# liuyuan-pal/NeRO

Measured on AMD Instinct MI355X. Metric: training rays/sec (Stage-I shape, 128 samples/ray), higher is better.
Workload: dtype f32 (dense layers: fp32 operands carried as exact / block-scaled 16-bit plane pairs or triples on the bf16/fp16 matrix pipe with fp32 accumulation, fp32-grade error; modes {'fwd': 'f16x3', 'tan': 'f16x3', 'bwd': 'f16x3', 'dw': 'f16x3'}); 1 GPU; GlossySynthetic 'bell' Stage-I shape, 4096 rays x (64+64+32) samples per GPU, training-schedule step 25000; rays_per_gpu=4096, parallelism=dp1, optimizer=adam(fused), streams=3, f16_paired_mask=3, fg_table=reference asset (tests/golden/fg_lut_ref.npz)

## Files before the change

### nero_amd/chain.py

```python
import ctypes as C
import os
import math

import torch

from . import _lib as L




_MODE_NAMES = {'f32': L.GEMM_F32, 'bf16x6': L.GEMM_BF16X6, 'f16x3': L.GEMM_F16X3}
_F16 = (L.GEMM_F16X3,)
_DEFAULT = {'fwd': 'f16x3', 'tan': 'f16x3', 'bwd': 'f16x3', 'dw': 'f16x3'}


def _resolve(mode, k):
    if mode not in _MODE_NAMES:
        raise ValueError(f"NERO_GEMM{'_' + k.upper()}: unknown arithmetic {mode!r} (one of {sorted(_MODE_NAMES)}; 'f16x3p' is not an arithmetic any more: "
                         "NERO_F16_PAIRED selects the workgroup organisation, DESIGN.md 9.3)")
    return _MODE_NAMES[mode]


GEMM_MODE = {k: _resolve(os.environ.get('NERO_GEMM_' + k.upper(), os.environ.get('NERO_GEMM', _DEFAULT[k])), k)
             for k in ('fwd', 'tan', 'bwd', 'dw')}
# ... 141 lines not shown
                e['hw'] = 4 * L.HID
                e['hb'] = 4
            sizes.append(e)
        return sizes

    def pack_floats(self):
        return sum(sum(e.values()) for e in self._sizes())

    def pack(self, buf=None, run=True):
        sizes = self._sizes()
        total = sum(sum(e.values()) for e in sizes)
        if buf is None:
            buf = torch.zeros(total, dtype=torch.float32, device=self.device)
        assert buf.numel() >= total
        off = 0
        packed = []
        jobs = []

        def job(kind, W, out, nrows, ld, col0, ncols, transpose, kpad, nt_count, scale=1.0):
            j = L.PackJob()
            j.W, j.out, j.kind, j.nrows, j.ld, j.col0, j.ncols = W.data_ptr(), out.data_ptr(), kind, nrows, ld, col0, ncols
            j.transpose, j.kpad, j.nt_count, j.scale = transpose, kpad, nt_count, scale
            jobs.append((j, W))

        for (d, h), e in zip(self.entries, sizes):
            p = {}
            for k, n in e.items():
                p[k] = buf[off:off + n] if n else None
                off += n
            if d is not None:
                W = d.W.detach()
                assert W.stride(1) == 1
                nt = _tiles(d.n_out)
                for key, c0, kc in (('fm', d.main_c0, d.k_main), ('fa', d.aux_c0, d.k_aux)):
                    if kc and key in p:
                        job(1, W, p[key], d.n_out, W.stride(0), c0, kc, 0, _r8(kc), nt, d.scale)
                for key, c0, kc in (('bm', d.main_c0, d.k_main), ('ba', d.aux_c0, d.k_aux)):
                    if kc and key in p:
                        job(1, W, p[key], d.n_out, W.stride(0), c0, kc, 1, _r8(d.n_out), _tiles(kc), d.scale)
                for key, c0, kc in (('sfm', d.main_c0, d.k_main), ('sfa', d.aux_c0, d.k_aux)):
                    if kc and key in p:
                        job(0, W, p[key], d.n_out, W.stride(0), c0, kc, 0, _r16(kc), nt, d.scale)
                for key, c0, kc in (('sbm', d.main_c0, d.k_main), ('sba', d.aux_c0, d.k_aux)):
                    if kc and key in p:
                        job(0, W, p[key], d.n_out, W.stride(0), c0, kc, 1, _r16(d.n_out), _tiles(kc), d.scale)
                for key, c0, kc in (('hfm', d.main_c0, d.k_main), ('hfa', d.aux_c0, d.k_aux)):
                    if kc and key in p:
                        job(3, W, p[key], d.n_out, W.stride(0), c0, kc, 0, _r16(kc), nt, d.scale)
                for key, c0, kc in (('hbm', d.main_c0, d.k_main), ('hba', d.aux_c0, d.k_aux)):
                    if kc and key in p:
                        job(3, W, p[key], d.n_out, W.stride(0), c0, kc, 1, _rev_k(d.n_out), _tiles(kc), d.scale)
                if d.b is not None:
                    b = d.b.detach()
                    job(2, b, p['bias'], 1, d.n_out, 0, d.n_out, 0, 32 * nt, 0)
            if h is not None:
                Wh = h.W.detach()
                assert Wh.stride(1) == 1
                job(2, Wh, p['hw'], h.n_head, Wh.stride(0), 0, h.k, 0, L.HID, 0)
                if h.b is not None:
                    job(2, h.b.detach(), p['hb'], 1, h.n_head, 0, h.n_head, 0, 4, 0)
            packed.append(p)
        self._packed, self._buf = packed, buf
        if not run:
            return jobs
        run_pack_jobs(jobs)
        return self

    def forward(self, init, aux, n_rows, save=True):
        assert self._packed is not None
        rp = row_pad(n_rows)
        ch = L.FwdChain()
        ch.init, ch.ld_init, ch.k_init = L.ptr(init), (init.stride(0) if init is not None else 0), self.k_init
        ch.aux, ch.ld_aux, ch.k_aux = L.ptr(aux), (aux.stride(0) if aux is not None else 0), self.k_aux
        ch.n_layers, ch.aux_wide = len(self.entries), int(self.aux_wide)
        split = GEMM_MODE['fwd'] != L.GEMM_F32
        fkeys = {L.GEMM_F32: ('fm', 'fa'), L.GEMM_BF16X6: ('sfm', 'sfa'), L.GEMM_F16X3: ('hfm', 'hfa')}[GEMM_MODE['fwd']]
        ch.gemm_mode = GEMM_MODE['fwd']
        ch.macs_per_row = float(sum(d.n_out * (d.k_main + d.k_aux) for d, _ in self.entries if d is not None))
        if init is not None:
            assert init.shape[0] >= rp and init.shape[1] >= self.k_init
        if aux is not None:
            assert aux.shape[0] >= rp and aux.shape[1] >= self.k_aux
        nd = len(self.dense_idx)
        last_dense = self.dense_idx[-1] if nd else -1
        saves, heads = [None] * len(self.entries), {}
        n_save = sum(1 for i in self.dense_idx if save or i == last_dense)
        sbuf = torch.empty((n_save, rp, L.HID), dtype=torch.float32, device=self.device)
        si = 0
        masks = [None] * len(self.entries)
        relu_idx = [i for i in self.dense_idx if save and self.entries[i][0].act == L.ACT_RELU] if GEMM_MODE['fwd'] in _F16 else []
        mbuf = torch.empty((len(relu_idx), rp, 8), dtype=torch.int32, device=self.device) if relu_idx else None
        for k, i in enumerate(relu_idx):
            masks[i] = mbuf[k]
        for i, ((d, h), p) in enumerate(zip(self.entries, self._packed)):
            fl = ch.layer[i]
            if h is not None:
                ho = torch.empty((rp, 4), dtype=torch.float32, device=self.device)
                heads[i] = ho
                fl.head_w, fl.head_b, fl.head_out = p['hw'].data_ptr(), p['hb'].data_ptr(), ho.data_ptr()
                fl.n_head, fl.head_k = h.n_head, (h.k + 3) // 4 * 4
            if d is not None:
                rk = _r16 if split else _r8
                fl.w_main = L.ptr(p.get(fkeys[0]))
                fl.w_aux = L.ptr(p.get(fkeys[1]))
                fl.bias = p['bias'].data_ptr()
                fl.k_main, fl.k_aux = (rk(d.k_main) if d.k_main else 0), (rk(d.k_aux) if d.k_aux else 0)
                fl.n_tiles, fl.act = _tiles(d.n_out), d.act
                if save or i == last_dense:
                    saves[i] = sbuf[si]
                    si += 1
                    fl.save = saves[i].data_ptr()
                if masks[i] is not None:
                    fl.relu_mask = masks[i].data_ptr()
        L.check(L.lib.nero_mlp_forward(C.byref(ch), n_rows, L.stream_ptr()))
        if MASK_CAPTURE is not None and relu_idx:
            MASK_CAPTURE.append({'k_init': self.k_init, 'k_aux': self.k_aux, 'aux_wide': bool(self.aux_wide), 'n_rows': n_rows,
                                 'n_out': [d.n_out if d is not None else 0 for d, _ in self.entries], 'masks': masks})
        return {'saves': saves, 'heads': heads, 'masks': masks, '_keep': (init, aux)}

    def backward(self, fwd, n_rows, dy=None, head_dys=None, need_dinit=False, need_daux=False, injs=None,
                 dinit_out=None, accumulate_dinit=False, skip_last_dense=False):
        head_dys = head_dys or {}
        injs = injs or {}
        rp = row_pad(n_rows)
        saves = fwd['saves']
        ch = L.BwdChain()
        ch.n_layers, ch.aux_wide = len(self.entries), 0
        split = GEMM_MODE['bwd'] != L.GEMM_F32
        bkeys = {L.GEMM_F32: ('bm', 'ba'), L.GEMM_BF16X6: ('sbm', 'sba'), L.GEMM_F16X3: ('hbm', 'hba')}[GEMM_MODE['bwd']]
        ch.gemm_mode = GEMM_MODE['bwd']
        rk = _r16 if split else _r8
        last = len(self.entries) - 1
        if dy is not None:
            ch.dy, ch.ld_dy = dy.data_ptr(), dy.stride(0)
            d_last = self.entries[last][0]
            ch.k_dy = _r8(d_last.n_out) if d_last is not None else L.HID
            assert dy.shape[1] >= ch.k_dy
        d_init = d_aux = None
        if need_dinit:
            d_init = dinit_out if dinit_out is not None else torch.empty((rp, self.k_init), dtype=torch.float32, device=self.device)
            ch.d_init, ch.ld_dinit, ch.accumulate_dinit = d_init.data_ptr(), d_init.stride(0), int(accumulate_dinit)
        if need_daux:
            d_aux = torch.zeros((rp, self.k_aux), dtype=torch.float32, device=self.device)
            ch.d_aux, ch.ld_daux = d_aux.data_ptr(), d_aux.stride(0)
        deltas = {}
        n_delta = len(self.dense_idx)
        dbuf = torch.empty((n_delta, rp, L.HID), dtype=torch.float32, device=self.device)
        prev_dense = {}
        pd = None
        for i, (d, h) in enumerate(self.entries):
            prev_dense[i] = pd
            if d is not None:
                pd = i
        for k, i in enumerate(self.dense_idx):
            deltas[i] = dbuf[k]
        for i, ((d, h), p) in enumerate(zip(self.entries, self._packed)):
            bl = ch.layer[i]
            j = prev_dense[i]
            if d is not None and not (skip_last_dense and i == last):
                bl.w_main_t = L.ptr(p.get(bkeys[0]))
                bl.w_aux_t = L.ptr(p.get(bkeys[1])) if need_daux else None
                bl.n_out = _rev_k(d.n_out) if GEMM_MODE['bwd'] in _F16 else rk(d.n_out)
                bl.k_main_tiles = _tiles(d.k_main) if d.k_main else 0
                bl.k_aux_tiles = _tiles(d.k_aux) if d.k_aux else 0
            else:
                bl.n_out = 0
                bl.k_main_tiles = _tiles(self.entries[j][0].n_out)
# ... 86 lines not shown
```

### nero_amd/csrc/chain_host.h

```cpp
#pragma once
#include <hip/hip_runtime_api.h>
#include <math.h>
#include <stdio.h>
#include <string.h>
#include <new>
#include <vector>
#include "../../include/nero_hip.h"

int nero_fail(int code, const char* msg);
int nero_check_launch(const char* what);
bool nero_prof_is_on();

namespace {

constexpr int MAXL = NERO_MAX_LAYERS;
inline int r8(int x) { return (x + 7) / 8 * 8; }
inline int r16(int x) { return (x + 15) / 16 * 16; }
inline int tiles(int x) { return (x + 31) / 32; }
inline int rpad(int n) { return NERO_ROW_PAD(n); }
inline int rev_k(int n_out) { return (n_out > 128 && n_out <= 256) ? 256 : r16(n_out); }
inline bool is_f16(int m) { return m == NERO_GEMM_F16X3; }

struct Arena {
    char* base = nullptr;
// ... 37 lines not shown
    float *bias = nullptr, *hfm = nullptr, *hfa = nullptr, *hbm = nullptr, *hba = nullptr, *hw = nullptr, *hb = nullptr;
};
struct Fwd {
    float* saves[MAXL]; uint32_t* masks[MAXL]; float* heads[MAXL];
    Fwd() { for (int i = 0; i < MAXL; ++i) { saves[i] = nullptr; masks[i] = nullptr; heads[i] = nullptr; } }
};
struct Bwd {
    const float* deltas[MAXL]; int ld_delta[MAXL];
    float* d_init = nullptr; int ld_dinit = 0; float* d_aux = nullptr; int ld_daux = 0;
    Bwd() { for (int i = 0; i < MAXL; ++i) { deltas[i] = nullptr; ld_delta[i] = NERO_HID; } }
};
struct Second { const float* D1 = nullptr; int ldd1 = 0; const float* B1m = nullptr; int ldb1m = 0; const float* B1a = nullptr; int ldb1a = 0; };

struct Modes { int fwd, tan, bwd, dw; };

struct Chain {
    std::vector<Entry> e;
    int k_init = 0, k_aux = 0, aux_wide = 0;
    int n() const { return (int)e.size(); }
    int last_dense() const { int l = -1; for (int i = 0; i < n(); ++i) if (e[i].d.has) l = i; return l; }

    size_t pack_floats() const {
        size_t t = 0;
        for (const Entry& x : e) {
            if (x.d.has) {
                const Dense& d = x.d;
                const int nt = tiles(d.n_out);
                t += 32 * nt;
                if (d.k_main) t += 64 + (size_t)(r16(d.k_main) / 16) * nt * 512 + 64 + (size_t)(rev_k(d.n_out) / 16) * tiles(d.k_main) * 512;
                if (d.k_aux) t += 64 + (size_t)(r16(d.k_aux) / 16) * nt * 512 + 64 + (size_t)(rev_k(d.n_out) / 16) * tiles(d.k_aux) * 512;
            }
            if (x.h.has) t += 4 * NERO_HID + 4;
        }
        return t;
    }
    void pack(float*& buf, std::vector<nero_pack_job>& jobs) {
        auto job = [&](int kind, const float* W, float* out, int nrows, int ld, int col0, int ncols, int transpose, int kpad, int nt_count, float scale) {
            nero_pack_job j;
            j.W = W; j.out = out; j.kind = kind; j.nrows = nrows; j.ld = ld; j.col0 = col0; j.ncols = ncols; j.transpose = transpose;
            j.kpad = kpad; j.nt_count = nt_count; j.scale = scale; j.pad_ = 0;
            jobs.push_back(j);
        };
        for (Entry& x : e) {
            if (x.d.has) {
                const Dense& d = x.d;
                const int nt = tiles(d.n_out);
                x.bias = buf; buf += 32 * nt;
                x.hfm = x.hfa = x.hbm = x.hba = nullptr;
                if (d.k_main) {
                    x.hfm = buf; buf += 64 + (size_t)(r16(d.k_main) / 16) * nt * 512;
                    x.hbm = buf; buf += 64 + (size_t)(rev_k(d.n_out) / 16) * tiles(d.k_main) * 512;
                    job(3, d.W, x.hfm, d.n_out, d.ldw, d.main_c0, d.k_main, 0, r16(d.k_main), nt, d.scale);
                    job(3, d.W, x.hbm, d.n_out, d.ldw, d.main_c0, d.k_main, 1, rev_k(d.n_out), tiles(d.k_main), d.scale);
                }
                if (d.k_aux) {
                    x.hfa = buf; buf += 64 + (size_t)(r16(d.k_aux) / 16) * nt * 512;
                    x.hba = buf; buf += 64 + (size_t)(rev_k(d.n_out) / 16) * tiles(d.k_aux) * 512;
                    job(3, d.W, x.hfa, d.n_out, d.ldw, d.aux_c0, d.k_aux, 0, r16(d.k_aux), nt, d.scale);
                    job(3, d.W, x.hba, d.n_out, d.ldw, d.aux_c0, d.k_aux, 1, rev_k(d.n_out), tiles(d.k_aux), d.scale);
                }
                if (d.b) job(2, d.b, x.bias, 1, d.n_out, 0, d.n_out, 0, 32 * nt, 0, 1.f);
            }
            if (x.h.has) {
                x.hw = buf; buf += 4 * NERO_HID;
                x.hb = buf; buf += 4;
                job(2, x.h.W, x.hw, x.h.n_head, x.h.ldw, 0, x.h.k, 0, NERO_HID, 0, 1.f);
                if (x.h.b) job(2, x.h.b, x.hb, 1, x.h.n_head, 0, x.h.n_head, 0, 4, 0, 1.f);
            }
        }
    }

    int forward(Arena& A, const Modes& M, const float* init, int ld_init, const float* aux, int ld_aux, int n_rows, bool save, Fwd& F,
                void* stream) const {
        const int rp = rpad(n_rows);
        nero_fwd_chain ch;
        memset(&ch, 0, sizeof(ch));
        ch.init = init; ch.ld_init = init ? ld_init : 0; ch.k_init = k_init;
        ch.aux = aux; ch.ld_aux = aux ? ld_aux : 0; ch.k_aux = k_aux;
        ch.n_layers = n(); ch.aux_wide = aux_wide;
        ch.gemm_mode = M.fwd;
        double macs = 0.0;
        for (const Entry& x : e) if (x.d.has) macs += (double)x.d.n_out * (x.d.k_main + x.d.k_aux);
        ch.macs_per_row = macs;
        const int ld = last_dense();
        for (int i = 0; i < n(); ++i) {
            const Entry& x = e[i];
            nero_fwd_layer& fl = ch.layer[i];
            if (x.h.has) {
                F.heads[i] = A.f32((size_t)rp * 4);
                fl.head_w = x.hw; fl.head_b = x.hb; fl.head_out = F.heads[i];
                fl.n_head = x.h.n_head; fl.head_k = (x.h.k + 3) / 4 * 4;
            }
            if (x.d.has) {
                const Dense& d = x.d;
                fl.w_main = x.hfm; fl.w_aux = x.hfa; fl.bias = x.bias;
                fl.k_main = d.k_main ? r16(d.k_main) : 0; fl.k_aux = d.k_aux ? r16(d.k_aux) : 0;
                fl.n_tiles = tiles(d.n_out); fl.act = d.act;
                if (save || i == ld) { F.saves[i] = A.f32((size_t)rp * NERO_HID); fl.save = F.saves[i]; }
                if (save && d.act == NERO_ACT_RELU) { F.masks[i] = reinterpret_cast<uint32_t*>(A.i32((size_t)rp * 8)); fl.relu_mask = F.masks[i]; }
            }
        }
        if (A.failed) return nero_fail(NERO_ERR_ARG, "nero_stage1: workspace too small");
        LAUNCH(nero_mlp_forward(&ch, n_rows, stream));
        return NERO_OK;
    }

    int backward(Arena& A, const Modes& M, const Fwd& F, int n_rows, const float* dy, int ld_dy, const float* const* head_dys ,
                 bool need_dinit, bool need_daux, const float* const* injs , float* dinit_out, int ld_dinit_out,
                 bool accumulate_dinit, bool skip_last_dense, Bwd& B, void* stream,
                 const float* const* inj_adots = nullptr ) const {
        const int rp = rpad(n_rows), last = n() - 1;
        nero_bwd_chain ch;
        memset(&ch, 0, sizeof(ch));
        ch.n_layers = n(); ch.aux_wide = 0; ch.gemm_mode = M.bwd;
        if (dy) {
            ch.dy = dy; ch.ld_dy = ld_dy;
            ch.k_dy = e[last].d.has ? r8(e[last].d.n_out) : NERO_HID;
        }
        if (need_dinit) {
            if (dinit_out) { B.d_init = dinit_out; B.ld_dinit = ld_dinit_out; }
            else { B.d_init = A.f32((size_t)rp * k_init); B.ld_dinit = k_init; }
            ch.d_init = B.d_init; ch.ld_dinit = B.ld_dinit; ch.accumulate_dinit = accumulate_dinit ? 1 : 0;
        }
        if (need_daux) {
            B.d_aux = A.f32((size_t)rp * k_aux); B.ld_daux = k_aux;
            if (!A.dry && !A.failed) (void)hipMemsetAsync(B.d_aux, 0, (size_t)rp * k_aux * 4, (hipStream_t)stream);
            ch.d_aux = B.d_aux; ch.ld_daux = k_aux;
        }
        int prev_dense[MAXL];
        int pd = -1;
        for (int i = 0; i < n(); ++i) { prev_dense[i] = pd; if (e[i].d.has) pd = i; }
        float* dw[MAXL];
        for (int i = 0; i < n(); ++i) {
            dw[i] = nullptr;
            if (e[i].d.has) { dw[i] = A.f32((size_t)rp * NERO_HID); B.deltas[i] = dw[i]; B.ld_delta[i] = NERO_HID; }
        }
        double macs = 0.0;
        for (int i = 0; i < n(); ++i) {
            const Entry& x = e[i];
            nero_bwd_layer& bl = ch.layer[i];
            const int j = prev_dense[i];
            if (x.d.has && !(skip_last_dense && i == last)) {
                const Dense& d = x.d;
                bl.w_main_t = x.hbm;
                bl.w_aux_t = need_daux ? x.hba : nullptr;
                bl.n_out = rev_k(d.n_out);
                bl.k_main_tiles = d.k_main ? tiles(d.k_main) : 0;
                bl.k_aux_tiles = d.k_aux ? tiles(d.k_aux) : 0;
                const bool first = j < 0;
                if (first && !need_dinit) macs += (need_daux && d.k_aux) ? (double)d.n_out * d.k_aux : 0.0;
                else macs += (double)d.n_out * (d.k_main + (need_daux ? d.k_aux : 0));
            } else {
                bl.n_out = 0;
                bl.k_main_tiles = j >= 0 ? tiles(e[j].d.n_out) : 0;
            }
            if (x.h.has && head_dys && head_dys[i]) { bl.head_w = x.hw; bl.head_dy = head_dys[i]; bl.n_head = x.h.n_head; }
            if (j >= 0) {
                bl.a_prev = F.saves[j];
                bl.act_prev = e[j].d.act;
                if (F.masks[j]) bl.mask_prev = F.masks[j];
                bl.delta_prev = dw[j];
                if (injs && injs[j]) { bl.inj = injs[j]; if (inj_adots && inj_adots[j]) bl.inj_adot = inj_adots[j]; }
            }
        }
        if (e[last].d.has && !skip_last_dense) { B.deltas[last] = dy; B.ld_delta[last] = ld_dy; }
        ch.macs_per_row = macs;
        if (A.failed) return nero_fail(NERO_ERR_ARG, "nero_stage1: workspace too small");
// ... 151 lines not shown
```

### nero_amd/csrc/mlp_f16_util.h

```cpp
#pragma once

#ifdef F16_PHASE_TIMING
__device__ unsigned long long g_phase[16];
#define PH_DECL long long ph_t = clock64(), ph_acc[8] = {0, 0, 0, 0, 0, 0, 0, 0}
#define PH(k) do { __builtin_amdgcn_sched_barrier(0); const long long t_ = clock64(); ph_acc[k] += t_ - ph_t; ph_t = t_; __builtin_amdgcn_sched_barrier(0); } while (0)
#define PH_PARAM , long long& ph_t, long long (&ph_acc)[8]
#define PH_ARG , ph_t, ph_acc
#define PH_END do { if (threadIdx.x == 0) for (int k_ = 0; k_ < 8; ++k_) atomicAdd(&g_phase[k_], (unsigned long long)ph_acc[k_]); } while (0)
#else
#define PH_PARAM
#define PH_ARG
#define PH_DECL
#define PH(k)
#define PH_END
#endif

typedef _Float16 f16x8 __attribute__((ext_vector_type(8)));
typedef _Float16 f16x2 __attribute__((ext_vector_type(2)));
typedef float f32x2 __attribute__((ext_vector_type(2)));
typedef float f32x16 __attribute__((ext_vector_type(16)));

constexpr float BETA = 100.0f;
constexpr int SA = 528;
constexpr int PLANE_A = 64 * SA;
// ... 303 lines not shown
                     "global_load_dwordx4 %2, %4, %6\n\tglobal_load_dwordx4 %3, %4, %6 offset:1024"
    if (ORDER_MEM) asm volatile(NERO_W2Q_ASM : "=&v"(o.ah), "=&v"(o.al), "=&v"(o.bh), "=&v"(o.bl) : "v"(voff), "s"(p0), "s"(p1) : "memory");
    else asm volatile(NERO_W2Q_ASM : "=&v"(o.ah), "=&v"(o.al), "=&v"(o.bh), "=&v"(o.bl) : "v"(voff), "s"(p0), "s"(p1));
#undef NERO_W2Q_ASM
}
static_assert(WQ_PLANE_BYTES == 1024, "offset:1024 in load_w2q");
template <int N> __device__ __forceinline__ void wait_vm() { asm volatile("s_waitcnt vmcnt(%0)" : : "n"(N)); }
__device__ __forceinline__ void landed_w2q(WQ2& w) {
    NERO_FENCE();
    asm volatile("" : "+v"(w.ah), "+v"(w.al), "+v"(w.bh), "+v"(w.bl));
}
__device__ __forceinline__ void ops_compute2q(f32x16 (&aH0)[2], f32x16 (&aH1)[2], const WQ2& w, const XF& x) {
    NERO_MFH(aH0[0], w.al, x.xh0); NERO_MFH(aH0[1], w.al, x.xh1);
    NERO_MFH(aH0[0], w.ah, x.xl0); NERO_MFH(aH0[1], w.ah, x.xl1);
    NERO_MFH(aH0[0], w.ah, x.xh0); NERO_MFH(aH0[1], w.ah, x.xh1);
    NERO_MFH(aH1[0], w.bl, x.xh0); NERO_MFH(aH1[1], w.bl, x.xh1);
    NERO_MFH(aH1[0], w.bh, x.xl0); NERO_MFH(aH1[1], w.bh, x.xl1);
    NERO_MFH(aH1[0], w.bh, x.xh0); NERO_MFH(aH1[1], w.bh, x.xh1);
}
__device__ __forceinline__ void prefill_w2q(WQ2& r0, WQ2& r1, unsigned voff, const char* s0, const char* s1) {
    load_w2q<0, true>(r0, voff, s0, s1);
    load_w2q<1, true>(r1, voff, s0, s1);
    NERO_FENCE();
}
constexpr int PRE_STORES = 2 * 2 * (32 / SCRP_ROWS) * (SCRP_ROWS / 8);
template <int N>
__device__ __forceinline__ void gemm_f16x3_dual_fixed(f32x16 (&aH0)[2], f32x16 (&aH1)[2], unsigned voff, const char* s0, const char* s1,
                                                      const char* xp, int half_bytes, int plane_bytes, WQ2& r0, WQ2& r1, bool stores_behind) {
    static_assert(N >= 3, "ring of three");
    WQ2 r2;
    XF x[2];
    load_x(x[0], xp, half_bytes, plane_bytes, 0);
    NERO_FENCE();
    static_for<0, N>([&](auto cc) {
        constexpr int c = cc.value;
        auto slot = [&](auto k) -> WQ2& { if constexpr (k.value % 3 == 0) return r0; else if constexpr (k.value % 3 == 1) return r1; else return r2; };
        if constexpr (c + 2 < N) load_w2q<c + 2, false>(slot(IC<c + 2>{}), voff, s0, s1);
        if constexpr (c + 1 < N) load_x(x[(c + 1) & 1], xp, half_bytes, plane_bytes, c + 1);
        NERO_FENCE();
        constexpr int later = 4 * ((c + 1 < N ? 1 : 0) + (c + 2 < N ? 1 : 0));
        if (c < 2 && stores_behind) wait_vm<later + PRE_STORES>();
        else wait_vm<later>();
        landed_w2q(slot(cc));
        ops_compute2q(aH0, aH1, slot(cc), x[c & 1]);
        NERO_FENCE();
    });
}

struct WQ1 { u32x4 h, l; };
template <int C> __device__ __forceinline__ void load_w1q(WQ1& o, unsigned voff, const char* s) {
    const char* p = s + C * WQ_STEP_BYTES;
    asm volatile("s_nop 4\n\tglobal_load_dwordx4 %0, %2, %3\n\tglobal_load_dwordx4 %1, %2, %3 offset:1024"
                 : "=&v"(o.h), "=&v"(o.l) : "v"(voff), "s"(p));
}
__device__ __forceinline__ void landed_w1q(WQ1& w) {
    NERO_FENCE();
    asm volatile("" : "+v"(w.h), "+v"(w.l));
}
template <int N>
__device__ __forceinline__ void gemm_f16x3_single_fixed(f32x16 (&aH)[2], unsigned voff, const char* s, const char* xp, int half_bytes,
                                                        int plane_bytes) {
    constexpr int WD = 3, WN = WD + 1;
    static_assert(N > WD, "ring of four");
    WQ1 w[WN];
    XF x[2];
    static_for<0, WD>([&](auto cc) { load_w1q<cc.value>(w[cc.value], voff, s); });
    load_x(x[0], xp, half_bytes, plane_bytes, 0);
    NERO_FENCE();
    static_for<0, N>([&](auto cc) {
        constexpr int c = cc.value;
        if constexpr (c + WD < N) load_w1q<c + WD>(w[(c + WD) % WN], voff, s);
        if constexpr (c + 1 < N) load_x(x[(c + 1) & 1], xp, half_bytes, plane_bytes, c + 1);
        NERO_FENCE();
        constexpr int later = 2 * ((c + 1 < N ? 1 : 0) + (c + 2 < N ? 1 : 0) + (c + 3 < N ? 1 : 0));
        wait_vm<later>();
        landed_w1q(w[c % WN]);
        NERO_MFH(aH[0], w[c % WN].l, x[c & 1].xh0); NERO_MFH(aH[1], w[c % WN].l, x[c & 1].xh1);
        NERO_MFH(aH[0], w[c % WN].h, x[c & 1].xl0); NERO_MFH(aH[1], w[c % WN].h, x[c & 1].xl1);
        NERO_MFH(aH[0], w[c % WN].h, x[c & 1].xh0); NERO_MFH(aH[1], w[c % WN].h, x[c & 1].xh1);
        NERO_FENCE();
    });
}

__device__ __forceinline__ void zero2(f32x16 (&acc)[2]) {
#pragma unroll
    for (int r = 0; r < 2; ++r)
#pragma unroll
        for (int v = 0; v < 16; ++v) acc[r][v] = 0.f;
}

template <int ACT>
__device__ __forceinline__ void fwd_values(const f32x16 (&aH)[2], const float4 (&bq)[4], const float (&U)[2], float4 (&val)[2][4],
                                           float (&m)[2]) {
#pragma unroll
    for (int r = 0; r < 2; ++r) {
        m[r] = 0.f;
#pragma unroll
        for (int g = 0; g < 4; ++g) {
            float4 v;
            v.x = act_fwd<ACT>(fmaf(aH[r][4 * g], U[r], bq[g].x));
            v.y = act_fwd<ACT>(fmaf(aH[r][4 * g + 1], U[r], bq[g].y));
            v.z = act_fwd<ACT>(fmaf(aH[r][4 * g + 2], U[r], bq[g].z));
            v.w = act_fwd<ACT>(fmaf(aH[r][4 * g + 3], U[r], bq[g].w));
            val[r][g] = v;
            m[r] = fmaxf(m[r], amax4(v));
        }
    }
}

__device__ __forceinline__ float max_xor32(float m) {
    const auto r = __builtin_amdgcn_permlane32_swap(__float_as_uint(m), __float_as_uint(m), false, false);
    return fmaxf(__uint_as_float(r[0]), __uint_as_float(r[1]));
}
__device__ __forceinline__ unsigned other_half(unsigned v, int h) {
    const auto r = __builtin_amdgcn_permlane32_swap(v, v, false, false);
    return h ? r[0] : r[1];
}
template <int CTRL> __device__ __forceinline__ float dpp_f32(float v) {
    return __uint_as_float(__builtin_amdgcn_update_dpp(0u, __float_as_uint(v), CTRL, 0xf, 0xf, true));
}
__device__ __forceinline__ float max_4lanes(float m) { m = fmaxf(m, dpp_f32<0xB1>(m)); return fmaxf(m, dpp_f32<0x4E>(m)); }
__device__ __forceinline__ float max_8lanes(float m) { m = max_4lanes(m); return fmaxf(m, dpp_f32<0x141>(m)); }
__device__ __forceinline__ float sum_8lanes(float s) { s += dpp_f32<0xB1>(s); s += dpp_f32<0x4E>(s); return s + dpp_f32<0x141>(s); }

__device__ __forceinline__ void publish_rowmax(float* rmax, float m0, float m1, int wave, int i, int h) {
    m0 = max_xor32(m0);
    m1 = max_xor32(m1);
    if (h == 0) { rmax[i * 8 + wave] = m0; rmax[(32 + i) * 8 + wave] = m1; }
}
__device__ __forceinline__ float row_max8(const float* rmax, int row) {
    const float4 a = *reinterpret_cast<const float4*>(rmax + row * 8);
    const float4 b = *reinterpret_cast<const float4*>(rmax + row * 8 + 4);
    return fmaxf(fmaxf(fmaxf(a.x, a.y), fmaxf(a.z, a.w)), fmaxf(fmaxf(b.x, b.y), fmaxf(b.z, b.w)));
}

template <int ACT, bool HEAD, bool PRE>
__device__ __forceinline__ void bwd_values(const float4 (&gq)[2][4], const float4 (&pa)[2][4], size_t goff, bool has_inj,
                                           const nero_bwd_layer& L, int row0, int i, int fbase, int n_rows, float4 (&val)[2][4],
                                           float (&m)[2], const float4 (&ijp)[2][4]) {
    const int nh = L.n_head;
    float4 gs[2][4];
#pragma unroll
    for (int r = 0; r < 2; ++r)
#pragma unroll
        for (int g = 0; g < 4; ++g) gs[r][g] = gq[r][g];
    if (HEAD) {
        float dj[2][4];
#pragma unroll
        for (int r = 0; r < 2; ++r) {
            const float4 dyh = *reinterpret_cast<const float4*>(L.head_dy + (size_t)(row0 + 32 * r + i) * 4);
            dj[r][0] = dyh.x; dj[r][1] = dyh.y; dj[r][2] = dyh.z; dj[r][3] = dyh.w;
        }
#pragma unroll
        for (int g = 0; g < 4; ++g) {
            float4 hw[4];
#pragma unroll
            for (int j = 0; j < 4; ++j) hw[j] = *reinterpret_cast<const float4*>(L.head_w + (j < nh ? j : 0) * NERO_HID + fbase + 8 * g);
#pragma unroll
            for (int r = 0; r < 2; ++r)
#pragma unroll
                for (int j = 0; j < 4; ++j)
                    if (j < nh) {
                        gs[r][g].x = fmaf(dj[r][j], hw[j].x, gs[r][g].x); gs[r][g].y = fmaf(dj[r][j], hw[j].y, gs[r][g].y);
                        gs[r][g].z = fmaf(dj[r][j], hw[j].z, gs[r][g].z); gs[r][g].w = fmaf(dj[r][j], hw[j].w, gs[r][g].w);
                    }
            __builtin_amdgcn_sched_barrier(0);
// ... 48 lines not shown
```

### nero_amd/csrc/mlp_f16x3.hip

```cpp
#include <hip/hip_runtime.h>
#include <stdint.h>
#include <stdlib.h>
#include "../../include/nero_hip.h"
#include "common.h"
#include "mlp_split.h"

namespace {

#include "mlp_f16_util.h"


__device__ __forceinline__ void acc_to_global(float* scr, const float4 (&q)[4], float* __restrict__ gblock, int lane) {
    const int i = lane & 31, h = lane >> 5;
#pragma unroll
    for (int g = 0; g < 4; ++g) *reinterpret_cast<float4*>(scr + i * SCR_LD + 8 * g + 4 * h) = q[g];
    __builtin_amdgcn_wave_barrier();
#pragma unroll
    for (int p = 0; p < 4; ++p)
        store_ws4(gblock + (size_t)(8 * p + (lane >> 3)) * NERO_HID + 4 * (lane & 7),
                  *reinterpret_cast<const float4*>(scr + (8 * p + (lane >> 3)) * SCR_LD + 4 * (lane & 7)));
    __builtin_amdgcn_wave_barrier();
}

template <int NV>
__device__ __forceinline__ void tile_request(float4 (&v)[NV], const float* __restrict__ src, int ld, int k, int row0, int n_rows, int tid) {
    const int r = tid >> 3, q = tid & 7;
    int gr = row0 + r;
    gr = gr < n_rows ? gr : n_rows - 1;
    const float* rowp = src + (size_t)gr * ld;
#pragma unroll
    for (int j = 0; j < NV; ++j) {
        const int c4 = 4 * (q + 8 * j);
        v[j] = make_float4(0.f, 0.f, 0.f, 0.f);
        if (c4 < k) v[j] = *reinterpret_cast<const float4*>(rowp + c4);
    }
}
template <int NV>
__device__ __forceinline__ void tile_commit(char* planes, int stride, int plane_bytes, float* rs, const float4 (&v)[NV], int k, int tid) {
    const int r = tid >> 3, q = tid & 7;
    const int k16 = (k + 15) & ~15, q4 = k16 >> 2;
    float m = 0.f;
#pragma unroll
    for (int j = 0; j < NV; ++j) m = fmaxf(m, fmaxf(fmaxf(fabsf(v[j].x), fabsf(v[j].y)), fmaxf(fabsf(v[j].z), fabsf(v[j].w))));
    m = max_8lanes(m);
    const int e = scale_exp(m);
    const float inv = pow2i(-e);
#pragma unroll
    for (int j = 0; j < NV; ++j) {
        const int c4 = 4 * (q + 8 * j);
        if (q + 8 * j < q4) {
            const float4 s = make_float4(v[j].x * inv, v[j].y * inv, v[j].z * inv, v[j].w * inv);
            store_planes4h(planes + r * stride + c4 * 2, plane_bytes, s);
        }
    }
    if (q == 0) rs[r] = pow2i(e);
}
__device__ __forceinline__ void load_planes_scaled(char* planes, int stride, int plane_bytes, float* rs, const float* __restrict__ src,
                                                   int ld, int k, int row0, int n_rows, int tid) {
    float4 v[8];
    tile_request<8>(v, src, ld, k, row0, n_rows, tid);
    tile_commit<8>(planes, stride, plane_bytes, rs, v, k, tid);
}

__device__ __forceinline__ void eval_head_f16(const char* planes, const float* rs, const float* __restrict__ w, const float* __restrict__ b,
                                              float* __restrict__ out, int n_head, int hk, int row0, int tid) {
    const int r = tid >> 3, q = tid & 7;
    float s[4] = {0.f, 0.f, 0.f, 0.f};
    float bj[4] = {0.f, 0.f, 0.f, 0.f};
    if (b) {
#pragma unroll
        for (int j = 0; j < 4; ++j) bj[j] = b[j < n_head ? j : 0];
    }
    for (int c4 = 4 * q; c4 < hk; c4 += 32) {
        const float4 x = load_planes4h(planes + r * SA + c4 * 2, PLANE_A);
        float4 ww[4];
#pragma unroll
        for (int j = 0; j < 4; ++j) ww[j] = *reinterpret_cast<const float4*>(w + (j < n_head ? j : 0) * NERO_HID + c4);
#pragma unroll
        for (int j = 0; j < 4; ++j) s[j] = fmaf(x.x, ww[j].x, fmaf(x.y, ww[j].y, fmaf(x.z, ww[j].z, fmaf(x.w, ww[j].w, s[j]))));
    }
#pragma unroll
    for (int j = 0; j < 4; ++j) s[j] = sum_8lanes(s[j]);
    if (q == 0) {
        const float sc = rs[r];
#pragma unroll
        for (int j = 0; j < 4; ++j)
            if (j < n_head) out[(size_t)(row0 + r) * 4 + j] = s[j] * sc + bj[j];
    }
}

struct Lds {
    char* actp; char* auxp; float* rs_main; float* rs_aux; float* rmax; float* wsc; char* scr;
};
template <int SX>
__device__ __forceinline__ Lds carve(char* smem) {
    Lds l;
    l.actp = smem;
    l.auxp = smem + 2 * PLANE_A;
    char* p = l.auxp + 2 * 64 * SX;
    l.rs_main = reinterpret_cast<float*>(p);
    l.rs_aux = l.rs_main + 64;
    l.rmax = l.rs_aux + 64;
    l.wsc = l.rmax + 64 * 8;
    l.scr = reinterpret_cast<char*>(l.wsc + 32);
    return l;
}
inline int f16_lds_bytes(int wide) { return 2 * PLANE_A + 2 * 64 * (wide ? SX_W : SX_N) + LDS_SMALL_BYTES + 8 * SCR_BYTES; }
inline int tan_lds_bytes() { return 2 * PLANE_A + 2 * 64 * SX_N + LDS_SMALL_BYTES + 8 * 8192; }

template <bool WIDE, int NVI>
__global__ __launch_bounds__(512, 1) void fwd_f16_kernel(nero_fwd_chain ch, int n_rows, int n_tiles_total) {
    extern __shared__ __attribute__((aligned(16))) char smem[];
    constexpr int SX = WIDE ? SX_W : SX_N;
    constexpr int PLANE_X = 64 * SX;
    constexpr int NVX = WIDE ? 3 : 2;
    constexpr int NVR = NVI > 0 ? NVI : 1, NXR = NVI > 0 ? NVX : 1;
    const Lds S = carve<SX>(smem);
    const int tid = threadIdx.x, lane = tid & 63;
    const int wave = __builtin_amdgcn_readfirstlane(tid >> 6);
    const int i = lane & 31, h = lane >> 5;
    unsigned gmask = 0u;
    for (int l = 0; l < ch.n_layers; ++l) gmask |= (ch.layer[l].n_tiles > 0 ? 1u : 0u) << l;
    const int first_gemm = gmask ? __builtin_ctz(gmask) : 0, last_gemm = gmask ? 31 - __builtin_clz(gmask) : -1;
    WF pw0, pw1, pw2;
    auto prefetch_layer = [&](const nero_fwd_layer& Ln) {
        if (wave >= Ln.n_tiles) return;
        const int sx = Ln.k_aux >> 4, sm = Ln.k_main >> 4;
        const int n = sx > 0 ? sx : sm;
        if (n <= 0) return;
        const float* img = sx > 0 ? Ln.w_aux : Ln.w_main;
        const uint4* wp = reinterpret_cast<const uint4*>(reinterpret_cast<const char*>(img) + HDR_BYTES) + (size_t)wave * n * 128 + lane;
        const int last = n - 1;
        load_w(pw0, wp, 0);
        if (F16_PW_N > 1) load_w(pw1, wp, 1 < last ? 1 : last);
        if (F16_PW_N > 2) load_w(pw2, wp, 2 < last ? 2 : last);
    };
    float4 tin[NVR], tax[NXR];
    auto request_tile = [&](int t) {
        if (ch.init) tile_request<NVR>(tin, ch.init, ch.ld_init, ch.k_init, t * 64, n_rows, tid);
        if (ch.aux) tile_request<NXR>(tax, ch.aux, ch.ld_aux, ch.k_aux, t * 64, n_rows, tid);
    };
    int tile = blockIdx.x;
    if (tile >= n_tiles_total) return;
    if (NVI > 0) request_tile(tile);
    nero_fwd_layer Ln = load_layer(ch, first_gemm);
    int ln_idx = first_gemm;
    if (last_gemm >= 0) prefetch_layer(Ln);
    {
        WscRegs wr;
        wsc_request(wr, ch, [](const nero_fwd_layer& Lx, const float*& pm, const float*& pa) { pm = Lx.k_main > 0 && Lx.n_tiles > 0 ? Lx.w_main : nullptr; pa = Lx.k_aux > 0 && Lx.n_tiles > 0 ? Lx.w_aux : nullptr; });
        wsc_commit(S.wsc, wr, tid);
    }
    for (; tile < n_tiles_total; tile += gridDim.x) {
    const int row0 = tile * 64;
    PH_DECL;
    if (NVI > 0) {
        if (ch.init) tile_commit<NVR>(S.actp, SA, PLANE_A, S.rs_main, tin, ch.k_init, tid);
        if (ch.aux) tile_commit<NXR>(S.auxp, SX, PLANE_X, S.rs_aux, tax, ch.k_aux, tid);
    } else {
        if (ch.init) load_planes_scaled(S.actp, SA, PLANE_A, S.rs_main, ch.init, ch.ld_init, ch.k_init, row0, n_rows, tid);
        if (ch.aux) load_planes_scaled(S.auxp, SX, PLANE_X, S.rs_aux, ch.aux, ch.ld_aux, ch.k_aux, row0, n_rows, tid);
    }
    __syncthreads();
    PH(0);
    for (int l = 0; l < ch.n_layers; ++l) {
        nero_fwd_layer L;
        if (l == ln_idx) L = Ln; else L = load_layer(ch, l);
        if (L.n_head > 0) eval_head_f16(S.actp, S.rs_main, L.head_w, L.head_b, L.head_out, L.n_head, L.head_k, row0, tid);
        if (L.n_tiles == 0) continue;
        const bool live_wave = wave < L.n_tiles;
        f32x16 aH[2];
        zero2(aH);
        float4 bq[4];
#pragma unroll
        for (int g = 0; g < 4; ++g)
            bq[g] = (live_wave && L.bias) ? *reinterpret_cast<const float4*>(L.bias + 32 * wave + 8 * g + 4 * h) : make_float4(0.f, 0.f, 0.f, 0.f);
        float U[2] = {1.f, 1.f};
        PH(1);
        if (live_wave) {
            const int sm = L.k_main >> 4, sx = L.k_aux >> 4;
            if (sx > 0) {
                const float wsc = S.wsc[2 * l + 1];
                gemm_f16x3_loop(aH, reinterpret_cast<const uint4*>(reinterpret_cast<const char*>(L.w_aux) + HDR_BYTES) + (size_t)wave * sx * 128 + lane,
                                S.auxp + i * SX + 16 * h, 32 * SX, PLANE_X, sx, true, pw0, pw1, pw2);
                U[0] = wsc * S.rs_aux[i];
                U[1] = wsc * S.rs_aux[32 + i];
            }
            if (sm > 0) {
                const float wsc = S.wsc[2 * l];
                const float u0 = wsc * S.rs_main[i], u1 = wsc * S.rs_main[32 + i];
                if (sx > 0) {
                    const float r0 = U[0] / u0, r1 = U[1] / u1;
#pragma unroll
                    for (int v = 0; v < 16; ++v) { aH[0][v] *= r0; aH[1][v] *= r1; }
                }
                U[0] = u0;
                U[1] = u1;
                gemm_f16x3_loop(aH, reinterpret_cast<const uint4*>(reinterpret_cast<const char*>(L.w_main) + HDR_BYTES) + (size_t)wave * sm * 128 + lane,
                                S.actp + i * SA + 16 * h, 32 * SA, PLANE_A, sm, sx == 0, pw0, pw1, pw2);
            }
        }
        NERO_FENCE();
        if (l != last_gemm) {
            ln_idx = l + 1 + __builtin_ctz(gmask >> (l + 1));
            Ln = load_layer(ch, ln_idx);
            prefetch_layer(Ln);
        } else {
            if (NVI > 0 && tile + (int)gridDim.x < n_tiles_total) request_tile(tile + gridDim.x);
            ln_idx = first_gemm;
            Ln = load_layer(ch, ln_idx);
            prefetch_layer(Ln);
        }
        NERO_FENCE();
        float4 val[2][4];
        float m[2] = {0.f, 0.f};
        PH(2);
        if (live_wave) {
            if (L.act == NERO_ACT_RELU) fwd_values<NERO_ACT_RELU>(aH, bq, U, val, m);
            else if (L.act == NERO_ACT_SOFTPLUS100) fwd_values<NERO_ACT_SOFTPLUS100>(aH, bq, U, val, m);
            else fwd_values<NERO_ACT_NONE>(aH, bq, U, val, m);
            PH(3);
            if (L.save) {
                float* scr = reinterpret_cast<float*>(S.scr + wave * SCR_BYTES);
                float* sblock = L.save + (size_t)row0 * NERO_HID + 32 * wave;
                acc_to_global(scr, val[0], sblock, lane);
                acc_to_global(scr, val[1], sblock + (size_t)32 * NERO_HID, lane);
            }
            if (L.relu_mask) {
#pragma unroll
                for (int r = 0; r < 2; ++r) {
                    unsigned bits = 0u;
#pragma unroll
                    for (int g = 0; g < 4; ++g) {
                        bits |= (val[r][g].x > 0.f ? 1u : 0u) << (4 * g);
                        bits |= (val[r][g].y > 0.f ? 1u : 0u) << (4 * g + 1);
                        bits |= (val[r][g].z > 0.f ? 1u : 0u) << (4 * g + 2);
                        bits |= (val[r][g].w > 0.f ? 1u : 0u) << (4 * g + 3);
                    }
                    const unsigned other = other_half(bits, h);
                    if (h == 0) L.relu_mask[(size_t)(row0 + 32 * r + i) * 8 + wave] = bits | (other << 16);
                }
            }
        }
        PH(4);
        publish_rowmax(S.rmax, m[0], m[1], wave, i, h);
        __syncthreads();
        PH(5);
        {
            const int e0 = scale_exp(row_max8(S.rmax, i)), e1 = scale_exp(row_max8(S.rmax, 32 + i));
            if (live_wave) {
                const float inv0 = pow2i(-e0), inv1 = pow2i(-e1);
                char* dst = S.actp + i * SA + (32 * wave + 4 * h) * 2;
#pragma unroll
                for (int g = 0; g < 4; ++g) {
                    const float4 a = val[0][g], b = val[1][g];
                    store_planes4h(dst + 16 * g, PLANE_A, make_float4(a.x * inv0, a.y * inv0, a.z * inv0, a.w * inv0));
                    store_planes4h(dst + 32 * SA + 16 * g, PLANE_A, make_float4(b.x * inv1, b.y * inv1, b.z * inv1, b.w * inv1));
                }
            }
            if (wave == 0 && h == 0) { S.rs_main[i] = pow2i(e0); S.rs_main[32 + i] = pow2i(e1); }
        }
        PH(6);
        __syncthreads();
        PH(7);
    }
    PH_END;
    __syncthreads();
    }
}

__device__ __forceinline__ void commit_planes(const Lds& S, const float4 (&val)[2][4], float m0, float m1, bool live_wave, int wave,
                                              int i, int h) {
    publish_rowmax(S.rmax, m0, m1, wave, i, h);
    __syncthreads();
    const int e0 = scale_exp(row_max8(S.rmax, i)), e1 = scale_exp(row_max8(S.rmax, 32 + i));
    if (live_wave) {
        const float inv0 = pow2i(-e0), inv1 = pow2i(-e1);
        char* dst = S.actp + i * SA + (32 * wave + 4 * h) * 2;
#pragma unroll
        for (int g = 0; g < 4; ++g) {
            store_planes4h(dst + 16 * g, PLANE_A, scale4(val[0][g], inv0));
            store_planes4h(dst + 32 * SA + 16 * g, PLANE_A, scale4(val[1][g], inv1));
// ... 448 lines not shown
```

Before: 156,100 rays/s.

## Replace forward f16x3 GEMM loop with a four-slot weight prefetch ring

Swaps the forward chain's f16x3 inner GEMM for a rolled ring loop. Weights stream through four register slots with staggered vmcnt waits, and the main weights are prefetched after the aux GEMM ends. It also saves the last dense activation only when that dense layer is the final entry, which cuts a save buffer write for chains that end in a head. The rolled loop is meant to shrink code size and keep weight loads in flight, at the cost of loop overhead and runtime wait branching.

Result: no change. 156,500 rays/s, median of 4 (+0.2%).

```diff
diff --git a/nero_amd/chain.py b/nero_amd/chain.py
--- a/nero_amd/chain.py
+++ b/nero_amd/chain.py
@@ -247,7 +247,7 @@
         if aux is not None:
             assert aux.shape[0] >= rp and aux.shape[1] >= self.k_aux
         nd = len(self.dense_idx)
-        last_dense = self.dense_idx[-1] if nd else -1
+        last_dense = self.dense_idx[-1] if nd and self.dense_idx[-1] == len(self.entries) - 1 else -1
         saves, heads = [None] * len(self.entries), {}
         n_save = sum(1 for i in self.dense_idx if save or i == last_dense)
         sbuf = torch.empty((n_save, rp, L.HID), dtype=torch.float32, device=self.device)
diff --git a/nero_amd/csrc/chain_host.h b/nero_amd/csrc/chain_host.h
--- a/nero_amd/csrc/chain_host.h
+++ b/nero_amd/csrc/chain_host.h
@@ -143,7 +143,7 @@
         double macs = 0.0;
         for (const Entry& x : e) if (x.d.has) macs += (double)x.d.n_out * (x.d.k_main + x.d.k_aux);
         ch.macs_per_row = macs;
-        const int ld = last_dense();
+        const int ld = last_dense() == n() - 1 ? n() - 1 : -1;
         for (int i = 0; i < n(); ++i) {
             const Entry& x = e[i];
             nero_fwd_layer& fl = ch.layer[i];
diff --git a/nero_amd/csrc/mlp_f16_util.h b/nero_amd/csrc/mlp_f16_util.h
--- a/nero_amd/csrc/mlp_f16_util.h
+++ b/nero_amd/csrc/mlp_f16_util.h
@@ -409,6 +409,62 @@
     });
 }
 
+__device__ __forceinline__ void load_w1(WQ1& o, const char* s, unsigned voff, int c) {
+    const char* p = s + (size_t)c * WQ_STEP_BYTES + voff;
+    o.h = *reinterpret_cast<const u32x4*>(p);
+    o.l = *reinterpret_cast<const u32x4*>(p + WQ_PLANE_BYTES);
+}
+__device__ __forceinline__ void prefetch_w1(WQ1& r0, WQ1& r1, WQ1& r2, const char* s, unsigned voff, int n) {
+    const int last = n - 1;
+    load_w1(r0, s, voff, 0);
+    load_w1(r1, s, voff, 1 < last ? 1 : last);
+    load_w1(r2, s, voff, 2 < last ? 2 : last);
+}
+__device__ __forceinline__ void ops_compute1q(f32x16 (&aH)[2], const WQ1& w, const XF& x) {
+    NERO_MFH(aH[0], w.l, x.xh0); NERO_MFH(aH[1], w.l, x.xh1);
+    NERO_MFH(aH[0], w.h, x.xl0); NERO_MFH(aH[1], w.h, x.xl1);
+    NERO_MFH(aH[0], w.h, x.xh0); NERO_MFH(aH[1], w.h, x.xh1);
+}
+__device__ __forceinline__ void wait_ring(int ls) {
+    if (ls >= 3) wait_vm<6>();
+    else if (ls == 2) wait_vm<4>();
+    else if (ls == 1) wait_vm<2>();
+    else wait_vm<0>();
+}
+__device__ __forceinline__ void gemm_f16x3_ring(f32x16 (&aH)[2], unsigned voff, const char* s, const char* xp, int half_bytes,
+                                                int plane_bytes, int n, WQ1& r0, WQ1& r1, WQ1& r2) {
+    WQ1 r3;
+    XF x0, x1;
+    load_x(x0, xp, half_bytes, plane_bytes, 0);
+    landed_w1q(r0); landed_w1q(r1); landed_w1q(r2);
+    NERO_FENCE();
+    int callers = 1;
+    PIN_S(callers);
+#pragma clang loop unroll(disable)
+    for (int c = 0; c < n; c += 4) {
+        static_for<0, 4>([&](auto kk) {
+            constexpr int k = kk.value;
+            auto slot = [&](auto j) -> WQ1& {
+                if constexpr (j.value % 4 == 0) return r0; else if constexpr (j.value % 4 == 1) return r1;
+                else if constexpr (j.value % 4 == 2) return r2; else return r3;
+            };
+            auto xs = [&](auto j) -> XF& { if constexpr (j.value % 2 == 0) return x0; else return x1; };
+            if (c + k < n) {
+                if (c + k + 3 < n) load_w1q<k + 3>(slot(IC<k + 3>{}), voff, s);
+                if (c + k + 1 < n) load_x(xs(IC<k + 1>{}), xp, half_bytes, plane_bytes, k + 1);
+                NERO_FENCE();
+                if (!(k < 3 && callers)) wait_ring(n - 1 - (c + k));
+                landed_w1q(slot(kk));
+                ops_compute1q(aH, slot(kk), xs(kk));
+                NERO_FENCE();
+            }
+        });
+        s += 4 * WQ_STEP_BYTES;
+        xp += 4 * 32;
+        callers = 0;
+    }
+}
+
 __device__ __forceinline__ void zero2(f32x16 (&acc)[2]) {
 #pragma unroll
     for (int r = 0; r < 2; ++r)
diff --git a/nero_amd/csrc/mlp_f16x3.hip b/nero_amd/csrc/mlp_f16x3.hip
--- a/nero_amd/csrc/mlp_f16x3.hip
+++ b/nero_amd/csrc/mlp_f16x3.hip
@@ -87,6 +87,10 @@
         for (int j = 0; j < 4; ++j)
             if (j < n_head) out[(size_t)(row0 + r) * 4 + j] = s[j] * sc + bj[j];
     }
+}
+
+__device__ __forceinline__ const char* w_tile(const float* w, int t, int n) {
+    return reinterpret_cast<const char*>(w) + HDR_BYTES + (size_t)t * n * WQ_STEP_BYTES;
 }
 
 struct Lds {
@@ -119,21 +123,18 @@
     const int tid = threadIdx.x, lane = tid & 63;
     const int wave = __builtin_amdgcn_readfirstlane(tid >> 6);
     const int i = lane & 31, h = lane >> 5;
+    const unsigned voff = 16u * lane;
     unsigned gmask = 0u;
     for (int l = 0; l < ch.n_layers; ++l) gmask |= (ch.layer[l].n_tiles > 0 ? 1u : 0u) << l;
     const int first_gemm = gmask ? __builtin_ctz(gmask) : 0, last_gemm = gmask ? 31 - __builtin_clz(gmask) : -1;
-    WF pw0, pw1, pw2;
+    WQ1 pw0, pw1, pw2;
     auto prefetch_layer = [&](const nero_fwd_layer& Ln) {
         if (wave >= Ln.n_tiles) return;
         const int sx = Ln.k_aux >> 4, sm = Ln.k_main >> 4;
         const int n = sx > 0 ? sx : sm;
         if (n <= 0) return;
-        const float* img = sx > 0 ? Ln.w_aux : Ln.w_main;
-        const uint4* wp = reinterpret_cast<const uint4*>(reinterpret_cast<const char*>(img) + HDR_BYTES) + (size_t)wave * n * 128 + lane;
-        const int last = n - 1;
-        load_w(pw0, wp, 0);
-        if (F16_PW_N > 1) load_w(pw1, wp, 1 < last ? 1 : last);
-        if (F16_PW_N > 2) load_w(pw2, wp, 2 < last ? 2 : last);
+        static_assert(F16_PW_N == 3, "prefetch_w1 fills the ring's slots 0, 1, 2");
+        prefetch_w1(pw0, pw1, pw2, w_tile(sx > 0 ? Ln.w_aux : Ln.w_main, wave, n), voff, n);
     };
     float4 tin[NVR], tax[NXR];
     auto request_tile = [&](int t) {
@@ -181,8 +182,8 @@
             const int sm = L.k_main >> 4, sx = L.k_aux >> 4;
             if (sx > 0) {
                 const float wsc = S.wsc[2 * l + 1];
-                gemm_f16x3_loop(aH, reinterpret_cast<const uint4*>(reinterpret_cast<const char*>(L.w_aux) + HDR_BYTES) + (size_t)wave * sx * 128 + lane,
-                                S.auxp + i * SX + 16 * h, 32 * SX, PLANE_X, sx, true, pw0, pw1, pw2);
+                gemm_f16x3_ring(aH, voff, w_tile(L.w_aux, wave, sx), S.auxp + i * SX + 16 * h, 32 * SX, PLANE_X, sx, pw0, pw1, pw2);
+                if (sm > 0) prefetch_w1(pw0, pw1, pw2, w_tile(L.w_main, wave, sm), voff, sm);
                 U[0] = wsc * S.rs_aux[i];
                 U[1] = wsc * S.rs_aux[32 + i];
             }
@@ -196,8 +197,7 @@
                 }
                 U[0] = u0;
                 U[1] = u1;
-                gemm_f16x3_loop(aH, reinterpret_cast<const uint4*>(reinterpret_cast<const char*>(L.w_main) + HDR_BYTES) + (size_t)wave * sm * 128 + lane,
-                                S.actp + i * SA + 16 * h, 32 * SA, PLANE_A, sm, sx == 0, pw0, pw1, pw2);
+                gemm_f16x3_ring(aH, voff, w_tile(L.w_main, wave, sm), S.actp + i * SA + 16 * h, 32 * SA, PLANE_A, sm, pw0, pw1, pw2);
             }
         }
         NERO_FENCE();
```
